# lightly-ai/lightly-train

Measured on NVIDIA B200. Metric: images/sec ViT-S/16 DINOv2 training step (2g+8l crops, bs64/GPU), higher is better.
Workload: dtype bf16

## Files before the change

lightly_train_b200/csrc/attention_tc.cu:

```cuda
#include <cuda.h>
#include "common.cuh"
#include "../../include/b200dino.h"

namespace b200 {
namespace attn_tc {

static constexpr int HD = 64;
static constexpr int BLOCK_Q = 128;
static constexpr int TILE_BYTES = BLOCK_Q * 128;
static constexpr float kLog2e = 1.4426950408889634f;

__device__ __forceinline__ uint64_t smem_desc(uint32_t smem_addr, uint32_t lbo_bytes, uint32_t sbo_bytes) {
  uint64_t d = 0;
  d |= (uint64_t)((smem_addr & 0x3FFFF) >> 4);
  d |= (uint64_t)((lbo_bytes >> 4) & 0x3FFF) << 16;
  d |= (uint64_t)((sbo_bytes >> 4) & 0x3FFF) << 32;
  d |= (uint64_t)1 << 46;
  d |= (uint64_t)2 << 61;
  return d;
}
__device__ __forceinline__ uint32_t instr_desc(int m, int n, int a_mn, int b_mn) {
  uint32_t d = 0;
  d |= 1u << 4;
  d |= 1u << 7;
// ... 791 lines not shown
    const uint32_t id_dq = instr_desc(BLOCK_Q, HD, 0, 1);
    for (int t = 0; t < n_tiles; ++t) {
      const uint32_t ph = t & 1;
      const uint64_t dQt_k = smem_desc(s0 + C::OFF_Q + t * TILE_BYTES, 16, 1024);
      const uint64_t dQt_mn = smem_desc(s0 + C::OFF_Q + t * TILE_BYTES, 64 * 128, 1024);
      const uint64_t dOt_k = smem_desc(s0 + C::OFF_DO + t * TILE_BYTES, 16, 1024);
      const uint64_t dOt_mn = smem_desc(s0 + C::OFF_DO + t * TILE_BYTES, 64 * 128, 1024);
      if (t > 0) {
        mbar_wait(bar_free, ph ^ 1);
        tc_fence_after();
      }
      if (elect_one_sync()) {
#pragma unroll
        for (int ks = 0; ks < 4; ++ks)
          umma_f16(tmem_base + C::TM_SDP, dQt_k + (uint64_t)(ks * 2), dK_kmaj + (uint64_t)(ks * 2), id_s, ks > 0 ? 1u : 0u);
        umma_commit(bar_s);
      }
      __syncwarp();
      mbar_wait(bar_p, ph);
      tc_fence_after();
      if (elect_one_sync()) {
#pragma unroll 1
        for (int mt = 0; mt < C::MT; ++mt)
#pragma unroll 1
          for (int ks = 0; ks < 8; ++ks)
            umma_f16(tmem_base + C::TM_DV + mt * 64, dP_mn + (uint64_t)((mt * 2 * TILE_BYTES + ks * 2048) >> 4),
                     dOt_mn + (uint64_t)((ks * 2048) >> 4), id_kv, (t > 0 || ks > 0) ? 1u : 0u);
#pragma unroll
        for (int ks = 0; ks < 4; ++ks)
          umma_f16(tmem_base + C::TM_SDP, dOt_k + (uint64_t)(ks * 2), dV_kmaj + (uint64_t)(ks * 2), id_s, ks > 0 ? 1u : 0u);
        umma_commit(bar_dp);
      }
      __syncwarp();
      mbar_wait(bar_ds, ph);
      tc_fence_after();
      if (elect_one_sync()) {
#pragma unroll 1
        for (int mt = 0; mt < C::MT; ++mt)
#pragma unroll 1
          for (int ks = 0; ks < 8; ++ks)
            umma_f16(tmem_base + C::TM_DK + mt * 64, dP_mn + (uint64_t)((mt * 2 * TILE_BYTES + ks * 2048) >> 4),
                     dQt_mn + (uint64_t)((ks * 2048) >> 4), id_kv, (t > 0 || ks > 0) ? 1u : 0u);
#pragma unroll 1
        for (int ks = 0; ks < NKV16; ++ks)
          umma_f16(tmem_base + C::TM_SDP, dP_kmaj + (uint64_t)(((ks >> 2) * TILE_BYTES + (ks & 3) * 32) >> 4),
                   dK_mn + (uint64_t)((ks * 2048) >> 4), id_dq, ks > 0 ? 1u : 0u);
        umma_commit(bar_dq);
      }
      __syncwarp();
    }
  } else {
    const int g = warp >> 2, q = warp & 3;
    const int r = q * 32 + lane;
    const uint32_t tL = tmem_base + ((uint32_t)(q * 32) << 16);
    const float sl2 = scale * kLog2e;
    uint8_t* sP = smem + C::OFF_P;
    if (g < C::QT) {
      const int m = g * BLOCK_Q + r;
      float L = 0.f, D = 0.f;
      if (m < rows_valid) {
        const int im = m / N;
        L = lse[((size_t)(b0 + im) * h + head) * N + (m - im * N)] * kLog2e;
        const uint4* po = reinterpret_cast<const uint4*>(outp + (row0 + m) * ld_out + head * HD);
        const uint4* pd = reinterpret_cast<const uint4*>(dout + (row0 + m) * ld_out + head * HD);
#pragma unroll
        for (int i = 0; i < 8; ++i) {
          const uint4 a = __ldg(po + i), c = __ldg(pd + i);
          const uint32_t aa[4] = {a.x, a.y, a.z, a.w}, cc[4] = {c.x, c.y, c.z, c.w};
#pragma unroll
          for (int j = 0; j < 4; ++j) {
            const float2 x = unpack_bf16x2(aa[j]), y = unpack_bf16x2(cc[j]);
            D = fmaf(x.x, y.x, D);
            D = fmaf(x.y, y.y, D);
          }
        }
      }
      sL[m] = L;
      sD[m] = D;
    }
    if (threadIdx.x < 192) sC[threadIdx.x] = 0.f;
    named_bar_sync(1, C::WORKERS * 32);
    for (int t = 0; t < n_tiles; ++t) {
      const uint32_t ph = t & 1;
      const int m = t * BLOCK_Q + r;
      const bool row_ok = m < rows_valid;
      const int klo = min(m / N, n_img - 1) * N, khi = klo + N;
      const float L = sL[m], D = sD[m];
      const int nfull = (G == 1) ? N / 16 : 0;
      mbar_wait(bar_s, ph);
      tc_fence_after();
      if (g == 0) bwd_p_pass<C::qb(0), C::qb(1)>(tL + C::TM_SDP, sP, r, row_ok, klo, khi, nfull, sl2, L);
      else if (g == 1) bwd_p_pass<C::qb(1), C::qb(2)>(tL + C::TM_SDP, sP, r, row_ok, klo, khi, nfull, sl2, L);
      else if (NG == 4 && g == 2) bwd_p_pass<C::qb(NG == 4 ? 2 : 0), C::qb(NG == 4 ? 3 : 1)>(tL + C::TM_SDP, sP, r, row_ok, klo, khi, nfull, sl2, L);
      else if (NG == 4) bwd_p_pass<C::qb(NG == 4 ? 3 : 0), C::qb(NG == 4 ? 4 : 1)>(tL + C::TM_SDP, sP, r, row_ok, klo, khi, nfull, sl2, L);
      fence_proxy_async();
      tc_fence_before();
      __syncwarp();
      if (lane == 0) mbar_arrive(bar_p);
      mbar_wait(bar_dp, ph);
      tc_fence_after();
      if (g == 0) bwd_ds_pass<C::qb(0), C::qb(1)>(tL + C::TM_SDP, sP, r, D);
      else if (g == 1) bwd_ds_pass<C::qb(1), C::qb(2)>(tL + C::TM_SDP, sP, r, D);
      else if (NG == 4 && g == 2) bwd_ds_pass<C::qb(NG == 4 ? 2 : 0), C::qb(NG == 4 ? 3 : 1)>(tL + C::TM_SDP, sP, r, D);
      else if (NG == 4) bwd_ds_pass<C::qb(NG == 4 ? 3 : 0), C::qb(NG == 4 ? 4 : 1)>(tL + C::TM_SDP, sP, r, D);
      fence_proxy_async();
      tc_fence_before();
      __syncwarp();
      if (lane == 0) mbar_arrive(bar_ds);
      if (g == 0 || (NG == 4 && g == 1)) {
        mbar_wait(bar_dq, ph);
        tc_fence_after();
        __nv_bfloat16* grow = dqkv + (row0 + m) * ld_dtok + head * HD;
        if (NG == 2) drain_tile(tL + C::TM_SDP, scale, row_ok, grow, colsum ? sC : nullptr, lane);
        else drain_cols32(tL + C::TM_SDP, g, scale, row_ok, grow, colsum ? sC : nullptr, lane);
        tc_fence_before();
        __syncwarp();
        if (lane == 0) mbar_arrive(bar_free);
      }
    }
    mbar_wait(bar_dq, (n_tiles - 1) & 1);
    tc_fence_after();
    if (NG == 2 && C::MT == 1) {
      const bool ok = r < rows_valid;
      __nv_bfloat16* base = dqkv + (row0 + r) * ld_dtok + head * HD + (size_t)(1 + g) * h * HD;
      drain_tile(tL + (g ? C::TM_DV : C::TM_DK), g ? 1.f : scale, ok, base, colsum ? sC + 64 + 64 * g : nullptr, lane);
    } else if (NG == 2) {
      const int key = g * BLOCK_Q + r;
      const bool ok = key < rows_valid;
      __nv_bfloat16* base = dqkv + (row0 + key) * ld_dtok + head * HD;
      drain_tile(tL + C::TM_DK + g * 64, scale, ok, base + (size_t)h * HD, colsum ? sC + 64 : nullptr, lane);
      drain_tile(tL + C::TM_DV + g * 64, 1.f, ok, base + (size_t)2 * h * HD, colsum ? sC + 128 : nullptr, lane);
    } else {
      const int mt = g & 1, is_v = g >> 1;
      const int key = mt * BLOCK_Q + r;
      const bool ok = key < rows_valid;
      __nv_bfloat16* base = dqkv + (row0 + key) * ld_dtok + head * HD + (size_t)(1 + is_v) * h * HD;
      drain_tile(tL + (is_v ? C::TM_DV : C::TM_DK) + mt * 64, is_v ? 1.f : scale, ok, base, colsum ? sC + 64 + 64 * is_v : nullptr, lane);
    }
    named_bar_sync(1, C::WORKERS * 32);
    if (colsum && threadIdx.x < 192) {
      const int part = threadIdx.x >> 6, d = threadIdx.x & 63;
      atomicAdd(colsum + (size_t)part * h * HD + head * HD + d, sC[threadIdx.x]);
    }
  }

  tc_fence_before();
  __syncthreads();
  if (warp == CTRL) {
    tc_fence_after();
    tmem_dealloc(tmem_base, C::TMEM_COLS);
  }
}

typedef CUresult (*PFN_encodeTiled)(CUtensorMap*, CUtensorMapDataType, cuuint32_t, void*, const cuuint64_t*, const cuuint64_t*,
                                    const cuuint32_t*, const cuuint32_t*, CUtensorMapInterleave, CUtensorMapSwizzle,
                                    CUtensorMapL2promotion, CUtensorMapFloatOOBfill);
static PFN_encodeTiled encode_fn() {
  static PFN_encodeTiled fn = nullptr;
  if (!fn) {
    void* p = nullptr;
    cudaDriverEntryPointQueryResult qres;
    if (cudaGetDriverEntryPoint("cuTensorMapEncodeTiled", &p, cudaEnableDefault, &qres) == cudaSuccess && p) fn = (PFN_encodeTiled)p;
  }
  return fn;
}
static int tmap_rows(CUtensorMap* tm, const void* base, long long rows, long long cols, long long ld, int box_rows) {
  PFN_encodeTiled enc = encode_fn();
  if (!enc) return B200_ERR_DRIVER;
  cuuint64_t dims[2] = {(cuuint64_t)cols, (cuuint64_t)rows};
  cuuint64_t strides[1] = {(cuuint64_t)ld * 2};
  cuuint32_t box[2] = {64u, (cuuint32_t)box_rows};
  cuuint32_t estr[2] = {1, 1};
  CUresult r = enc(tm, CU_TENSOR_MAP_DATA_TYPE_BFLOAT16, 2, const_cast<void*>(base), dims, strides, box, estr,
                   CU_TENSOR_MAP_INTERLEAVE_NONE, CU_TENSOR_MAP_SWIZZLE_128B, CU_TENSOR_MAP_L2_PROMOTION_L2_256B,
                   CU_TENSOR_MAP_FLOAT_OOB_FILL_NONE);
  return r == CUDA_SUCCESS ? B200_OK : B200_ERR_DRIVER;
}

template <int NKV16>
static int launch_fwd(const void* qkv, long long ld_tok, int B, int N, int G, int h, float scale, void* out, long long ld_out,
                      float* lse, cudaStream_t s) {
  using C = FwdCfg<NKV16>;
  CUtensorMap tmQ, tmKV;
  int rc = tmap_rows(&tmQ, qkv, (long long)B * N, 3LL * h * HD, ld_tok, BLOCK_Q);
  if (rc) return rc;
  rc = tmap_rows(&tmKV, qkv, (long long)B * N, 3LL * h * HD, ld_tok, C::NKV);
  if (rc) return rc;
  static bool attr = false;
  if (!attr) {
    if (cudaFuncSetAttribute(attn_fwd_tc_kernel<NKV16>, cudaFuncAttributeMaxDynamicSharedMemorySize, C::SMEM_BYTES) != cudaSuccess)
      return B200_ERR_CUDA;
    attr = true;
  }
  launch_kernel(attn_fwd_tc_kernel<NKV16>, ((B + G - 1) / G) * h, C::THREADS, C::SMEM_BYTES, s, tmQ, tmKV, B, N, G, h, scale, (__nv_bfloat16*)out,
                                                                                  ld_out, lse);
  B200_CHECK_LAUNCH();
  return B200_OK;
}

template <int NKV16>
static int launch_fwd7(const void* qkv, long long ld_tok, int B, int N, int G, int h, float scale, void* out, long long ld_out,
                       float* lse, cudaStream_t s) {
  using C = Fwd7Cfg<NKV16>;
  CUtensorMap tmQ, tmKV;
  int rc = tmap_rows(&tmQ, qkv, (long long)B * N, 3LL * h * HD, ld_tok, BLOCK_Q);
  if (rc) return rc;
  rc = tmap_rows(&tmKV, qkv, (long long)B * N, 3LL * h * HD, ld_tok, C::NKV);
  if (rc) return rc;
  static bool attr = false;
  if (!attr) {
    if (cudaFuncSetAttribute(attn_fwd_tc7_kernel<NKV16>, cudaFuncAttributeMaxDynamicSharedMemorySize, C::SMEM_BYTES) != cudaSuccess)
      return B200_ERR_CUDA;
    attr = true;
  }
  const int tiles = (G * N + BLOCK_Q - 1) / BLOCK_Q;
  launch_kernel(attn_fwd_tc7_kernel<NKV16>, ((B + G - 1) / G) * h * tiles, C::THREADS, C::SMEM_BYTES, s, tmQ, tmKV, B, N, G, h, tiles,
                scale, (__nv_bfloat16*)out, ld_out, lse);
  B200_CHECK_LAUNCH();
  return B200_OK;
}

template <int NKV16>
static int launch_fwd8(const void* qkv, long long ld_tok, int B, int N, int G, int h, float scale, void* out, long long ld_out,
                       float* lse, cudaStream_t s) {
  using C = Fwd7Cfg<NKV16>;
  CUtensorMap tmQ, tmKV;
  int rc = tmap_rows(&tmQ, qkv, (long long)B * N, 3LL * h * HD, ld_tok, BLOCK_Q);
  if (rc) return rc;
  rc = tmap_rows(&tmKV, qkv, (long long)B * N, 3LL * h * HD, ld_tok, C::NKV);
  if (rc) return rc;
  static bool attr = false;
  static int num_sms = 0;
  if (!attr) {
    if (cudaFuncSetAttribute(attn_fwd_tc8_kernel<NKV16>, cudaFuncAttributeMaxDynamicSharedMemorySize, C::SMEM_BYTES) != cudaSuccess)
      return B200_ERR_CUDA;
    int dev = 0;
    cudaGetDevice(&dev);
    cudaDeviceGetAttribute(&num_sms, cudaDevAttrMultiProcessorCount, dev);
    attr = true;
  }
  const int tiles = (G * N + BLOCK_Q - 1) / BLOCK_Q;
  const int total = ((B + G - 1) / G) * h * tiles;
  const int grid = total < 2 * num_sms ? total : 2 * num_sms;
  launch_kernel(attn_fwd_tc8_kernel<NKV16>, grid, C::THREADS, C::SMEM_BYTES, s, tmQ, tmKV, B, N, G, h, tiles, total, scale,
                (__nv_bfloat16*)out, ld_out, lse);
  B200_CHECK_LAUNCH();
  return B200_OK;
}

template <int NKV16, int NG>
static int launch_bwd(const void* qkv, long long ld_tok, const void* out, const void* dout, long long ld_out, const float* lse, int B,
                      int N, int G, int h, float scale, void* dqkv, long long ld_dtok, float* colsum, cudaStream_t s) {
  using C = BwdCfg<NKV16, NG>;
  CUtensorMap tmQ, tmKV, tmDO;
  int rc = tmap_rows(&tmQ, qkv, (long long)B * N, 3LL * h * HD, ld_tok, BLOCK_Q);
  if (rc) return rc;
  rc = tmap_rows(&tmKV, qkv, (long long)B * N, 3LL * h * HD, ld_tok, C::NKV);
  if (rc) return rc;
  rc = tmap_rows(&tmDO, dout, (long long)B * N, (long long)h * HD, ld_out, BLOCK_Q);
  if (rc) return rc;
  static bool attr = false;
  if (!attr) {
    if (cudaFuncSetAttribute(attn_bwd_tc_kernel<NKV16, NG>, cudaFuncAttributeMaxDynamicSharedMemorySize, C::SMEM_BYTES) != cudaSuccess)
      return B200_ERR_CUDA;
    attr = true;
  }
  launch_kernel(attn_bwd_tc_kernel<NKV16, NG>, ((B + G - 1) / G) * h, C::THREADS, C::SMEM_BYTES, s, tmQ, tmKV, tmDO, (const __nv_bfloat16*)out,
                                                                                  (const __nv_bfloat16*)dout, ld_out, lse, B, N, G, h,
                                                                                  scale, (__nv_bfloat16*)dqkv, ld_dtok, colsum);
  B200_CHECK_LAUNCH();
  return B200_OK;
}

}
}

extern "C" int b200_attention_fwd_tc(const void* qkv, long long ld_tok, int B, int N, int h, int head_dim, float scale, void* out,
                                     long long ld_out, float* lse, void* stream) {
  using namespace b200::attn_tc;
  if (!qkv || !out || B <= 0 || N <= 0 || h <= 0 || !(scale > 0.f)) return B200_ERR_INVALID_ARG;
  if (head_dim != HD || (ld_tok % 8) || (ld_out % 8) || ((uintptr_t)qkv & 15) || ((uintptr_t)out & 15)) return B200_ERR_UNSUPPORTED;
  if (N > 256) return B200_ERR_UNSUPPORTED;
  cudaStream_t s = (cudaStream_t)stream;
  static int sched = -1;
  if (sched < 0) {
    const char* e = std::getenv("B200_ATTN_FWD_SCHEDULE");
    sched = (e && (e[0] == '1' || e[0] == '7' || e[0] == '8')) ? e[0] - '0' : 8;
  }
  if (sched == 8) {
    if (N <= 128) return launch_fwd8<8>(qkv, ld_tok, B, N, 128 / N, h, scale, out, ld_out, lse, s);
    if (N <= 208) return launch_fwd8<13>(qkv, ld_tok, B, N, 1, h, scale, out, ld_out, lse, s);
    return launch_fwd8<16>(qkv, ld_tok, B, N, 1, h, scale, out, ld_out, lse, s);
  }
  if (sched == 7) {
    if (N <= 128) return launch_fwd7<8>(qkv, ld_tok, B, N, 128 / N, h, scale, out, ld_out, lse, s);
    if (N <= 208) return launch_fwd7<13>(qkv, ld_tok, B, N, 1, h, scale, out, ld_out, lse, s);
    return launch_fwd7<16>(qkv, ld_tok, B, N, 1, h, scale, out, ld_out, lse, s);
  }
  if (N <= 128) return launch_fwd<8>(qkv, ld_tok, B, N, 128 / N, h, scale, out, ld_out, lse, s);
  if (N <= 208) return launch_fwd<13>(qkv, ld_tok, B, N, 1, h, scale, out, ld_out, lse, s);
  return launch_fwd<16>(qkv, ld_tok, B, N, 1, h, scale, out, ld_out, lse, s);
}

extern "C" int b200_attention_bwd_tc(const void* qkv, long long ld_tok, const void* out, const void* dout, long long ld_out,
                                     const float* lse, int B, int N, int h, int head_dim, float scale, void* dqkv,
                                     long long ld_dtok, float* dqkv_colsum, void* stream) {
  using namespace b200::attn_tc;
  if (!qkv || !out || !dout || !lse || !dqkv || B <= 0 || N <= 0 || h <= 0 || !(scale > 0.f)) return B200_ERR_INVALID_ARG;
  if (head_dim != HD || (ld_tok % 8) || (ld_out % 8) || (ld_dtok % 8)) return B200_ERR_UNSUPPORTED;
  if (((uintptr_t)qkv & 15) || ((uintptr_t)out & 15) || ((uintptr_t)dout & 15) || ((uintptr_t)dqkv & 15)) return B200_ERR_UNSUPPORTED;
  if (N > 208) return B200_ERR_UNSUPPORTED;
  cudaStream_t s = (cudaStream_t)stream;
  static int groups = -1;
  if (groups < 0) {
    const char* e = std::getenv("B200_ATTN_BWD_GROUPS");
    groups = (e && e[0] == '2') ? 2 : 4;
  }
  if (N <= 128) return launch_bwd<8, 2>(qkv, ld_tok, out, dout, ld_out, lse, B, N, 128 / N, h, scale, dqkv, ld_dtok, dqkv_colsum, s);
  if (groups == 4) {
    return launch_bwd<13, 4>(qkv, ld_tok, out, dout, ld_out, lse, B, N, 1, h, scale, dqkv, ld_dtok, dqkv_colsum, s);
  }
  return launch_bwd<13, 2>(qkv, ld_tok, out, dout, ld_out, lse, B, N, 1, h, scale, dqkv, ld_dtok, dqkv_colsum, s);
}
```

lightly_train_b200/csrc/common.cuh:

```cuda
#pragma once
#include <cuda_runtime.h>
#include <cuda_bf16.h>
#include <stdint.h>

#define B200_OK 0
#define B200_ERR_INVALID_ARG (-1)
#define B200_ERR_UNSUPPORTED (-2)
#define B200_ERR_CUDA (-3)
#define B200_ERR_DRIVER (-4)

#define B200_CHECK_LAUNCH()                                     \
  do {                                                          \
    cudaError_t e__ = cudaGetLastError();                       \
    if (e__ != cudaSuccess) return B200_ERR_CUDA - (int)e__ * 16; \
  } while (0)

#include <cstdlib>
#include <utility>

namespace b200 {

__device__ __forceinline__ void pdl_launch_dependents() { asm volatile("griddepcontrol.launch_dependents;"); }
__device__ __forceinline__ void pdl_wait() { asm volatile("griddepcontrol.wait;" ::: "memory"); }
#define B200_PDL_SYNC()                \
  do {                                 \
    b200::pdl_launch_dependents();     \
    b200::pdl_wait();                  \
  } while (0)

inline bool pdl_enabled() {
  static int v = -1;
  if (v < 0) {
    const char* e = std::getenv("B200_PDL");
    v = (e && e[0] == '1') ? 1 : 0;
  }
  return v == 1;
}

template <typename... KArgs, typename... Args>
inline void launch_kernel(void (*kernel)(KArgs...), dim3 grid, dim3 block, size_t smem, cudaStream_t stream, Args&&... args) {
  cudaLaunchConfig_t cfg = {};
  cfg.gridDim = grid;
  cfg.blockDim = block;
  cfg.dynamicSmemBytes = smem;
  cfg.stream = stream;
  cudaLaunchAttribute attr[1];
  attr[0].id = cudaLaunchAttributeProgrammaticStreamSerialization;
  attr[0].val.programmaticStreamSerializationAllowed = 1;
  cfg.attrs = attr;
  cfg.numAttrs = pdl_enabled() ? 1 : 0;
  (void)cudaLaunchKernelEx(&cfg, kernel, static_cast<KArgs>(std::forward<Args>(args))...);
}

__device__ __forceinline__ uint32_t smem_u32(const void* p) {
  return (uint32_t)__cvta_generic_to_shared(p);
}

__device__ __forceinline__ void mbar_init(uint64_t* bar, uint32_t count) {
  asm volatile("mbarrier.init.shared::cta.b64 [%0], %1;" ::"r"(smem_u32(bar)), "r"(count));
}
__device__ __forceinline__ void mbar_expect_tx(uint64_t* bar, uint32_t bytes) {
  asm volatile("mbarrier.arrive.expect_tx.shared::cta.b64 _, [%0], %1;" ::"r"(smem_u32(bar)),
               "r"(bytes)
               : "memory");
}
__device__ __forceinline__ void mbar_arrive(uint64_t* bar) {
  asm volatile("mbarrier.arrive.shared::cta.b64 _, [%0];" ::"r"(smem_u32(bar)) : "memory");
}
__device__ __forceinline__ bool mbar_try_wait(uint64_t* bar, uint32_t parity) {
  uint32_t ok;
  asm volatile(
      "{\n"
      ".reg .pred p;\n"
      "mbarrier.try_wait.parity.shared::cta.b64 p, [%1], %2;\n"
      "selp.u32 %0, 1, 0, p;\n"
      "}\n"
      : "=r"(ok)
      : "r"(smem_u32(bar)), "r"(parity)
      : "memory");
  return ok != 0;
}
__device__ __forceinline__ void mbar_wait(uint64_t* bar, uint32_t parity) {
  uint32_t spins = 0;
  while (!mbar_try_wait(bar, parity)) {
    if (++spins > (1u << 26)) __trap();
  }
}
__device__ __forceinline__ void fence_barrier_init() {
  asm volatile("fence.mbarrier_init.release.cluster;" ::: "memory");
}
__device__ __forceinline__ void fence_proxy_async() {
  asm volatile("fence.proxy.async.shared::cta;" ::: "memory");
}

__device__ __forceinline__ void tma_prefetch_desc(const void* tm) {
  asm volatile("prefetch.tensormap [%0];" ::"l"(tm) : "memory");
}
__device__ __forceinline__ void tma_load_2d(void* smem_dst, const void* tm, uint64_t* bar, int c0,
                                            int c1) {
  asm volatile(
      "cp.async.bulk.tensor.2d.shared::cluster.global.tile.mbarrier::complete_tx::bytes "
      "[%0], [%1, {%3, %4}], [%2];" ::"r"(smem_u32(smem_dst)),
      "l"(tm), "r"(smem_u32(bar)), "r"(c0), "r"(c1)
      : "memory");
}

__device__ __forceinline__ bool elect_one_sync() {
  uint32_t pred;
  asm volatile(
      "{\n"
      ".reg .pred p;\n"
      "elect.sync _|p, 0xffffffff;\n"
      "selp.u32 %0, 1, 0, p;\n"
      "}\n"
      : "=r"(pred));
  return pred != 0;
}

__device__ __forceinline__ void prefetch_l2(const void* p) {
  asm volatile("prefetch.global.L2 [%0];" ::"l"(p));
}

__device__ __forceinline__ void tmem_alloc(uint32_t* smem_dst, uint32_t ncols) {
  asm volatile("tcgen05.alloc.cta_group::1.sync.aligned.shared::cta.b32 [%0], %1;" ::"r"(
                   smem_u32(smem_dst)),
               "r"(ncols));
}
__device__ __forceinline__ void tmem_relinquish() {
  asm volatile("tcgen05.relinquish_alloc_permit.cta_group::1.sync.aligned;" ::);
}
__device__ __forceinline__ void tmem_dealloc(uint32_t taddr, uint32_t ncols) {
  asm volatile("tcgen05.dealloc.cta_group::1.sync.aligned.b32 %0, %1;" ::"r"(taddr), "r"(ncols));
}
__device__ __forceinline__ void tc_fence_before() {
  asm volatile("tcgen05.fence::before_thread_sync;" ::: "memory");
}
__device__ __forceinline__ void tc_fence_after() {
  asm volatile("tcgen05.fence::after_thread_sync;" ::: "memory");
}
__device__ __forceinline__ void umma_f16(uint32_t tmem_d, uint64_t adesc, uint64_t bdesc,
                                         uint32_t idesc, uint32_t accumulate) {
  asm volatile(
      "{\n"
      ".reg .pred p;\n"
      "setp.ne.b32 p, %4, 0;\n"
      "tcgen05.mma.cta_group::1.kind::f16 [%0], %1, %2, %3, p;\n"
      "}\n" ::"r"(tmem_d),
      "l"(adesc), "l"(bdesc), "r"(idesc), "r"(accumulate)
      : "memory");
}
__device__ __forceinline__ void umma_f16_ts(uint32_t tmem_d, uint32_t tmem_a, uint64_t bdesc, uint32_t idesc, uint32_t accumulate) {
  asm volatile(
      "{\n"
      ".reg .pred p;\n"
      "setp.ne.b32 p, %4, 0;\n"
      "tcgen05.mma.cta_group::1.kind::f16 [%0], [%1], %2, %3, p;\n"
      "}\n" ::"r"(tmem_d),
      "r"(tmem_a), "l"(bdesc), "r"(idesc), "r"(accumulate)
      : "memory");
}
__device__ __forceinline__ void umma_commit(uint64_t* bar) {
  asm volatile("tcgen05.commit.cta_group::1.mbarrier::arrive::one.shared::cluster.b64 [%0];" ::"r"(
                   smem_u32(bar))
               : "memory");
}
__device__ __forceinline__ uint32_t cluster_ctarank() {
  uint32_t r;
  asm volatile("mov.u32 %0, %%cluster_ctarank;" : "=r"(r));
  return r;
}
__device__ __forceinline__ void cluster_sync_all() {
  asm volatile("barrier.cluster.arrive.release.aligned;\nbarrier.cluster.wait.acquire.aligned;" ::: "memory");
}
__device__ __forceinline__ uint32_t mapa_u32(uint32_t smem_addr, uint32_t rank) {
  uint32_t r;
  asm volatile("mapa.shared::cluster.u32 %0, %1, %2;" : "=r"(r) : "r"(smem_addr), "r"(rank));
  return r;
}
__device__ __forceinline__ void mbar_arrive_cluster(uint32_t cluster_addr) {
  asm volatile("mbarrier.arrive.shared::cluster.b64 _, [%0];" ::"r"(cluster_addr) : "memory");
}
__device__ __forceinline__ void tma_load_2d_2sm(void* smem_dst, const void* tm, uint32_t bar_cluster_addr, int c0, int c1) {
  asm volatile(
      "cp.async.bulk.tensor.2d.cta_group::2.shared::cluster.global.tile.mbarrier::complete_tx::bytes "
      "[%0], [%1, {%3, %4}], [%2];" ::"r"(smem_u32(smem_dst)),
      "l"(tm), "r"(bar_cluster_addr), "r"(c0), "r"(c1)
      : "memory");
}
__device__ __forceinline__ void tmem_alloc_2sm(uint32_t* smem_dst, uint32_t ncols) {
  asm volatile("tcgen05.alloc.cta_group::2.sync.aligned.shared::cta.b32 [%0], %1;" ::"r"(smem_u32(smem_dst)), "r"(ncols));
}
__device__ __forceinline__ void tmem_relinquish_2sm() {
  asm volatile("tcgen05.relinquish_alloc_permit.cta_group::2.sync.aligned;" ::);
}
__device__ __forceinline__ void tmem_dealloc_2sm(uint32_t taddr, uint32_t ncols) {
  asm volatile("tcgen05.dealloc.cta_group::2.sync.aligned.b32 %0, %1;" ::"r"(taddr), "r"(ncols));
}
__device__ __forceinline__ void umma_f16_2sm(uint32_t tmem_d, uint64_t adesc, uint64_t bdesc, uint32_t idesc,
                                             uint32_t accumulate) {
  asm volatile(
      "{\n"
      ".reg .pred p;\n"
      "setp.ne.b32 p, %4, 0;\n"
      "tcgen05.mma.cta_group::2.kind::f16 [%0], %1, %2, %3, p;\n"
      "}\n" ::"r"(tmem_d),
      "l"(adesc), "l"(bdesc), "r"(idesc), "r"(accumulate)
      : "memory");
}
__device__ __forceinline__ void umma_commit_2sm(uint64_t* bar, uint16_t cta_mask) {
  asm volatile("tcgen05.commit.cta_group::2.mbarrier::arrive::one.shared::cluster.multicast::cluster.b64 [%0], %1;" ::"r"(
                   smem_u32(bar)),
               "h"(cta_mask)
               : "memory");
}

__device__ __forceinline__ void tmem_ld_32x32(uint32_t taddr, uint32_t (&v)[32]) {
  asm volatile(
      "tcgen05.ld.sync.aligned.32x32b.x32.b32 "
      "{%0, %1, %2, %3, %4, %5, %6, %7, %8, %9, %10, %11, %12, %13, %14, %15, "
      "%16, %17, %18, %19, %20, %21, %22, %23, %24, %25, %26, %27, %28, %29, %30, %31}, [%32];"
      : "=r"(v[0]), "=r"(v[1]), "=r"(v[2]), "=r"(v[3]), "=r"(v[4]), "=r"(v[5]), "=r"(v[6]),
        "=r"(v[7]), "=r"(v[8]), "=r"(v[9]), "=r"(v[10]), "=r"(v[11]), "=r"(v[12]), "=r"(v[13]),
        "=r"(v[14]), "=r"(v[15]), "=r"(v[16]), "=r"(v[17]), "=r"(v[18]), "=r"(v[19]), "=r"(v[20]),
        "=r"(v[21]), "=r"(v[22]), "=r"(v[23]), "=r"(v[24]), "=r"(v[25]), "=r"(v[26]), "=r"(v[27]),
        "=r"(v[28]), "=r"(v[29]), "=r"(v[30]), "=r"(v[31])
      : "r"(taddr));
}
__device__ __forceinline__ void tmem_ld_32x16(uint32_t taddr, uint32_t (&v)[16]) {
  asm volatile(
      "tcgen05.ld.sync.aligned.32x32b.x16.b32 "
      "{%0, %1, %2, %3, %4, %5, %6, %7, %8, %9, %10, %11, %12, %13, %14, %15}, [%16];"
      : "=r"(v[0]), "=r"(v[1]), "=r"(v[2]), "=r"(v[3]), "=r"(v[4]), "=r"(v[5]), "=r"(v[6]), "=r"(v[7]), "=r"(v[8]),
        "=r"(v[9]), "=r"(v[10]), "=r"(v[11]), "=r"(v[12]), "=r"(v[13]), "=r"(v[14]), "=r"(v[15])
      : "r"(taddr));
}
__device__ __forceinline__ void tmem_ld_32x8(uint32_t taddr, uint32_t (&v)[8]) {
  asm volatile("tcgen05.ld.sync.aligned.32x32b.x8.b32 {%0, %1, %2, %3, %4, %5, %6, %7}, [%8];"
               : "=r"(v[0]), "=r"(v[1]), "=r"(v[2]), "=r"(v[3]), "=r"(v[4]), "=r"(v[5]), "=r"(v[6]), "=r"(v[7])
               : "r"(taddr));
}
__device__ __forceinline__ void tmem_ld_wait() {
  asm volatile("tcgen05.wait::ld.sync.aligned;" ::: "memory");
}
__device__ __forceinline__ void tmem_st_32x8(uint32_t taddr, const uint32_t (&v)[8]) {
  asm volatile("tcgen05.st.sync.aligned.32x32b.x8.b32 [%0], {%1, %2, %3, %4, %5, %6, %7, %8};" ::"r"(taddr), "r"(v[0]), "r"(v[1]),
               "r"(v[2]), "r"(v[3]), "r"(v[4]), "r"(v[5]), "r"(v[6]), "r"(v[7])
               : "memory");
}
__device__ __forceinline__ void tmem_st_wait() {
  asm volatile("tcgen05.wait::st.sync.aligned;" ::: "memory");
}

__device__ __forceinline__ float bf16_round(float x) {
  return __bfloat162float(__float2bfloat16_rn(x));
}
__device__ __forceinline__ uint32_t pack_bf16x2(float lo, float hi) {
  __nv_bfloat162 h = __floats2bfloat162_rn(lo, hi);
  return *reinterpret_cast<uint32_t*>(&h);
}
// ... 75 lines not shown
```

Before: 3437.

## Add persistent pipelined attention backward kernel with TMEM-resident P and dS

Adds a new persistent attention backward kernel, enabled by default, that loops over (image group, head) pairs with a grid capped at the SM count. It keeps P and dS in tensor memory for the TS-form MMAs, double-buffers LSE and D, prefetches the next pair's tiles to L2 with TMA, and uses separate drain warps to overlap the dK/dV/dQ writeback with the next tile's work. The aim is to cut launch and tail overhead and the serialization between softmax-gradient math and tensor-core work. The cost is a much more complex mbarrier protocol with more room for ordering bugs, and tighter TMEM and shared-memory budgets.

```diff
diff --git a/lightly_train_b200/csrc/attention_tc.cu b/lightly_train_b200/csrc/attention_tc.cu
--- a/lightly_train_b200/csrc/attention_tc.cu
+++ b/lightly_train_b200/csrc/attention_tc.cu
@@ -967,6 +967,426 @@
   }
 }
 
+template <int NKV16>
+struct Bwd2Cfg {
+  static constexpr int NKV = NKV16 * 16;
+  static constexpr bool SMALL = NKV <= 128;
+  static constexpr int MT = SMALL ? 1 : 2;
+  static constexpr int NG = SMALL ? 2 : 4;
+  static constexpr int Q_BYTES = NKV * 128;
+  static constexpr int OFF_Q = 0;
+  static constexpr int OFF_DO = Q_BYTES;
+  static constexpr int OFF_K = 2 * Q_BYTES;
+  static constexpr int OFF_V = OFF_K + MT * TILE_BYTES;
+  static constexpr int OFF_DS = OFF_V + MT * TILE_BYTES;
+  static constexpr int OFF_F = OFF_DS + 2 * MT * TILE_BYTES;
+  static constexpr int OFF_BAR = OFF_F + (4 * 256 + 192) * 4;
+  static constexpr int SMEM_BYTES = OFF_BAR + 128 + 1024;
+  static constexpr int WORKERS = 4 * NG;
+  static constexpr int DRAIN = WORKERS;
+  static constexpr int CTRL = WORKERS + 4;
+  static constexpr int THREADS = (WORKERS + 5) * 32;
+  static constexpr int CTAS_PER_SM = SMALL ? 2 : 1;
+  static constexpr int TP = 0;
+  static constexpr int TDP = (NKV / 2 + 15) / 16 * 16;
+  static constexpr int TDS = TDP;
+  static constexpr int TDK = (TDP + NKV / 2 + 31) / 32 * 32;
+  static constexpr int TDV = TDP + NKV;
+  static constexpr int TDQ = SMALL ? 0 : TDV + 64;
+  static constexpr int TMEM_COLS = SMALL ? 256 : 512;
+  __host__ __device__ static constexpr int qb(int g) { return (NKV16 * g + NG - 1) / NG; }
+  static_assert(TDK + 64 <= TDP + NKV && TDV + 64 <= TMEM_COLS && TDQ + 64 * MT <= TMEM_COLS, "TMEM column plan");
+  static_assert(SMALL ? TDQ + 64 <= TDP : TDQ >= TDV + 64, "dQ overlaps only P^T (packed) or nothing (global)");
+  static_assert(CTAS_PER_SM * SMEM_BYTES <= 232448, "shared memory");
+};
+
+template <int NT>
+__device__ __forceinline__ void quarter_bar_sync(int q) {
+  switch (q) {
+    case 0: asm volatile("bar.sync 1, %0;" ::"n"(NT) : "memory"); break;
+    case 1: asm volatile("bar.sync 2, %0;" ::"n"(NT) : "memory"); break;
+    case 2: asm volatile("bar.sync 3, %0;" ::"n"(NT) : "memory"); break;
+    default: asm volatile("bar.sync 4, %0;" ::"n"(NT) : "memory"); break;
+  }
+}
+
+template <int NKV16, int C0, int C1>
+__device__ __forceinline__ void bwd2_p_pass(uint32_t tL, int qq, const float* L, bool key_ok, int qlo, int qhi, int nfull, float sl2) {
+  using C = Bwd2Cfg<NKV16>;
+  constexpr int NC = C1 - C0;
+  uint32_t sv[NC * 8];
+  uint32_t buf[16];
+  tmem_ld_32x16(tL + C0 * 16, buf);
+#pragma unroll
+  for (int c = 0; c < NC; ++c) {
+    tmem_ld_wait();
+#pragma unroll
+    for (int i = 0; i < 8; ++i) sv[c * 8 + i] = pack_bf16x2(__uint_as_float(buf[2 * i]), __uint_as_float(buf[2 * i + 1]));
+    if (c + 1 < NC) tmem_ld_32x16(tL + (C0 + c + 1) * 16, buf);
+  }
+  tc_fence_before();
+  quarter_bar_sync<C::NG * 32>(qq);
+  tc_fence_after();
+  const float kb = key_ok ? 0.f : -INFINITY;
+#pragma unroll
+  for (int c = 0; c < NC; ++c) {
+    const int q0 = (C0 + c) * 16;
+    uint32_t pw[8];
+    if (C0 + c < nfull) {
+#pragma unroll
+      for (int i = 0; i < 8; ++i) {
+        const float2 ss = unpack_bf16x2(sv[c * 8 + i]);
+        const float2 ll = *reinterpret_cast<const float2*>(L + q0 + 2 * i);
+        pw[i] = pack_bf16x2(ex2_ftz(fmaf(ss.x, sl2, kb - ll.x)), ex2_ftz(fmaf(ss.y, sl2, kb - ll.y)));
+      }
+    } else {
+#pragma unroll
+      for (int i = 0; i < 8; ++i) {
+        const float2 ss = unpack_bf16x2(sv[c * 8 + i]);
+        const float2 ll = *reinterpret_cast<const float2*>(L + q0 + 2 * i);
+        const int q = q0 + 2 * i;
+        const float p0 = (key_ok && q >= qlo && q < qhi) ? ex2_ftz(fmaf(ss.x, sl2, -ll.x)) : 0.f;
+        const float p1 = (key_ok && q + 1 >= qlo && q + 1 < qhi) ? ex2_ftz(fmaf(ss.y, sl2, -ll.y)) : 0.f;
+        pw[i] = pack_bf16x2(p0, p1);
+      }
+    }
+    tmem_st_32x8(tL + C::TP + (C0 + c) * 8, pw);
+  }
+  tmem_st_wait();
+}
+
+template <int NKV16, int C0, int C1>
+__device__ __forceinline__ void bwd2_ds_pass(uint32_t tL, int qq, const float* Dq, uint8_t* sDS, int r) {
+  using C = Bwd2Cfg<NKV16>;
+  constexpr int NC = C1 - C0;
+  uint32_t dv[NC * 8];
+  uint32_t buf[16];
+  tmem_ld_32x16(tL + C::TDP + C0 * 16, buf);
+#pragma unroll
+  for (int c = 0; c < NC; ++c) {
+    tmem_ld_wait();
+#pragma unroll
+    for (int i = 0; i < 8; ++i) dv[c * 8 + i] = pack_bf16x2(__uint_as_float(buf[2 * i]), __uint_as_float(buf[2 * i + 1]));
+    if (c + 1 < NC) tmem_ld_32x16(tL + C::TDP + (C0 + c + 1) * 16, buf);
+  }
+  uint32_t pk[8];
+  tmem_ld_32x8(tL + C::TP + C0 * 8, pk);
+  tc_fence_before();
+  quarter_bar_sync<C::NG * 32>(qq);
+  tc_fence_after();
+#pragma unroll
+  for (int c = 0; c < NC; ++c) {
+    tmem_ld_wait();
+    uint32_t pc[8];
+#pragma unroll
+    for (int i = 0; i < 8; ++i) pc[i] = pk[i];
+    if (c + 1 < NC) tmem_ld_32x8(tL + C::TP + (C0 + c + 1) * 8, pk);
+    const int q0 = (C0 + c) * 16;
+    uint32_t dw[8];
+#pragma unroll
+    for (int i = 0; i < 8; ++i) {
+      const float2 dp = unpack_bf16x2(dv[c * 8 + i]);
+      const float2 pp = unpack_bf16x2(pc[i]);
+      const float2 dd = *reinterpret_cast<const float2*>(Dq + q0 + 2 * i);
+      dw[i] = pack_bf16x2(pp.x * (dp.x - dd.x), pp.y * (dp.y - dd.y));
+    }
+    tmem_st_32x8(tL + C::TDS + (C0 + c) * 8, dw);
+    uint8_t* slab = sDS + ((C0 + c) >> 2) * TILE_BYTES;
+    const int ch = ((C0 + c) & 3) * 2;
+    *reinterpret_cast<uint4*>(slab + swz(r, ch)) = make_uint4(dw[0], dw[1], dw[2], dw[3]);
+    *reinterpret_cast<uint4*>(slab + swz(r, ch + 1)) = make_uint4(dw[4], dw[5], dw[6], dw[7]);
+  }
+  tmem_st_wait();
+}
+
+template <int MT>
+__device__ __forceinline__ void bwd2_drain_dq(uint32_t tdq, int r, int rows_valid, float scale, __nv_bfloat16* dq_rows, long long ld_dtok,
+                                              float* cs, int lane, uint64_t* bar_dqfree) {
+#pragma unroll 1
+  for (int mq = 0; mq < MT; ++mq)
+    drain_tile(tdq + mq * 64, scale, mq * BLOCK_Q + r < rows_valid, dq_rows + (size_t)mq * BLOCK_Q * ld_dtok, cs, lane);
+  tc_fence_before();
+  __syncwarp();
+  if (lane == 0) mbar_arrive(bar_dqfree);
+}
+
+template <int NKV16>
+__global__ void __launch_bounds__(Bwd2Cfg<NKV16>::THREADS, Bwd2Cfg<NKV16>::CTAS_PER_SM)
+attn_bwd_tc2_kernel(const __grid_constant__ CUtensorMap tmQ, const __grid_constant__ CUtensorMap tmKV,
+                    const __grid_constant__ CUtensorMap tmDO, const __nv_bfloat16* __restrict__ outp,
+                    const __nv_bfloat16* __restrict__ dout, long long ld_out, const float* __restrict__ lse, int B, int N, int G,
+                    int h, int n_pairs, float scale, __nv_bfloat16* __restrict__ dqkv, long long ld_dtok, float* __restrict__ colsum) {
+  pdl_launch_dependents();
+  using C = Bwd2Cfg<NKV16>;
+  constexpr int MT = C::MT;
+  extern __shared__ uint8_t smem_raw[];
+  uint8_t* smem = reinterpret_cast<uint8_t*>((reinterpret_cast<uintptr_t>(smem_raw) + 1023) & ~(uintptr_t)1023);
+  float* sL = reinterpret_cast<float*>(smem + C::OFF_F);
+  float* sD = sL + 512;
+  float* sC = sD + 512;
+  uint64_t* bars = reinterpret_cast<uint64_t*>(smem + C::OFF_BAR);
+  uint64_t* bar_qd = bars + 0;
+  uint64_t* bar_kv = bars + 1;
+  uint64_t* bar_s = bars + 3;
+  uint64_t* bar_p = bars + 4;
+  uint64_t* bar_dp = bars + 5;
+  uint64_t* bar_ds = bars + 6;
+  uint64_t* bar_dk = bars + 7;
+  uint64_t* bar_kvfree = bars + 8;
+  uint64_t* bar_dqfree = bars + 9;
+  uint32_t* tmem_slot = reinterpret_cast<uint32_t*>(bars + 10);
+
+  const int warp = threadIdx.x >> 5, lane = threadIdx.x & 31;
+  if (threadIdx.x == 0) {
+    mbar_init(bar_qd, 1);
+    for (int kt = 0; kt < MT; ++kt) mbar_init(bar_kv + kt, 1);
+    mbar_init(bar_s, 1);
+    mbar_init(bar_p, C::WORKERS);
+    mbar_init(bar_dp, 1);
+    mbar_init(bar_ds, C::WORKERS);
+    mbar_init(bar_dk, 1);
+    mbar_init(bar_kvfree, 4);
+    mbar_init(bar_dqfree, 4);
+    fence_barrier_init();
+  }
+  if (threadIdx.x < 192) sC[threadIdx.x] = 0.f;
+  if (warp == C::CTRL) {
+    if (lane == 0) {
+      tma_prefetch_desc(&tmQ);
+      tma_prefetch_desc(&tmKV);
+      tma_prefetch_desc(&tmDO);
+    }
+    tmem_alloc(tmem_slot, C::TMEM_COLS);
+    tmem_relinquish();
+  }
+  tc_fence_before();
+  __syncthreads();
+  tc_fence_after();
+  pdl_wait();
+  const uint32_t tmem_base = *tmem_slot;
+  const int n_mine = (n_pairs - (int)blockIdx.x + (int)gridDim.x - 1) / (int)gridDim.x;
+  auto pair_coords = [h, G](int it, int& head, int& b0) {
+    const int w = blockIdx.x + it * gridDim.x;
+    head = w % h;
+    b0 = (w / h) * G;
+  };
+
+  if (warp == C::CTRL) {
+    const uint32_t s0 = smem_u32(smem);
+    const uint64_t dQ_k = smem_desc(s0 + C::OFF_Q, 16, 1024);
+    const uint64_t dO_k = smem_desc(s0 + C::OFF_DO, 16, 1024);
+    const uint64_t dQ_mn = smem_desc(s0 + C::OFF_Q, 64 * 128, 1024);
+    const uint64_t dO_mn = smem_desc(s0 + C::OFF_DO, 64 * 128, 1024);
+    const uint32_t id_s = instr_desc(BLOCK_Q, C::NKV, 0, 0);
+    const uint32_t id_ts = instr_desc(BLOCK_Q, HD, 0, 1);
+    const uint32_t id_dq = instr_desc(BLOCK_Q, HD, 1, 1);
+    auto load_qd = [&](int it) {
+      int head, b0;
+      pair_coords(it, head, b0);
+      mbar_expect_tx(bar_qd, 2 * C::Q_BYTES);
+      tma_load_2d(smem + C::OFF_Q, &tmQ, bar_qd, head * HD, b0 * N);
+      tma_load_2d(smem + C::OFF_DO, &tmDO, bar_qd, head * HD, b0 * N);
+    };
+    auto load_kv = [&](int it, int kt) {
+      int head, b0;
+      pair_coords(it, head, b0);
+      mbar_expect_tx(bar_kv + kt, 2 * TILE_BYTES);
+      tma_load_2d(smem + C::OFF_K + kt * TILE_BYTES, &tmKV, bar_kv + kt, (h + head) * HD, b0 * N + kt * BLOCK_Q);
+      tma_load_2d(smem + C::OFF_V + kt * TILE_BYTES, &tmKV, bar_kv + kt, (2 * h + head) * HD, b0 * N + kt * BLOCK_Q);
+    };
+    if (lane == 0 && n_mine > 0) {
+      load_qd(0);
+      for (int kt = 0; kt < MT; ++kt) load_kv(0, kt);
+    }
+    __syncwarp();
+    for (int it = 0; it < n_mine; ++it) {
+      for (int kt = 0; kt < MT; ++kt) {
+        const int j = it * MT + kt;
+        if (kt == 0) {
+          mbar_wait(bar_qd, it & 1);
+          if (lane == 0 && it + 1 < n_mine) {
+            int head, b0;
+            pair_coords(it + 1, head, b0);
+            tma_prefetch_2d(&tmQ, head * HD, b0 * N);
+            tma_prefetch_2d(&tmDO, head * HD, b0 * N);
+            for (int k2 = 0; k2 < MT; ++k2) {
+              tma_prefetch_2d(&tmKV, (h + head) * HD, b0 * N + k2 * BLOCK_Q);
+              tma_prefetch_2d(&tmKV, (2 * h + head) * HD, b0 * N + k2 * BLOCK_Q);
+            }
+          }
+          __syncwarp();
+        }
+        mbar_wait(bar_kv + kt, it & 1);
+        if (C::SMALL && it > 0) mbar_wait(bar_dqfree, (it - 1) & 1);
+        tc_fence_after();
+        if (elect_one_sync()) {
+          const uint64_t dK_k = smem_desc(s0 + C::OFF_K + kt * TILE_BYTES, 16, 1024);
+#pragma unroll
+          for (int ks = 0; ks < HD / 16; ++ks)
+            umma_f16(tmem_base, dK_k + (uint64_t)(ks * 2), dQ_k + (uint64_t)(ks * 2), id_s, ks > 0 ? 1u : 0u);
+          umma_commit(bar_s);
+        }
+        __syncwarp();
+        mbar_wait(bar_p, j & 1);
+        if (j > 0) mbar_wait(bar_kvfree, (j - 1) & 1);
+        tc_fence_after();
+        if (elect_one_sync()) {
+#pragma unroll 1
+          for (int ks = 0; ks < NKV16; ++ks)
+            umma_f16_ts(tmem_base + C::TDV, tmem_base + C::TP + ks * 8, dO_mn + (uint64_t)((ks * 2048) >> 4), id_ts, ks > 0 ? 1u : 0u);
+          const uint64_t dV_k = smem_desc(s0 + C::OFF_V + kt * TILE_BYTES, 16, 1024);
+#pragma unroll
+          for (int ks = 0; ks < HD / 16; ++ks)
+            umma_f16(tmem_base + C::TDP, dV_k + (uint64_t)(ks * 2), dO_k + (uint64_t)(ks * 2), id_s, ks > 0 ? 1u : 0u);
+          umma_commit(bar_dp);
+        }
+        __syncwarp();
+        mbar_wait(bar_ds, j & 1);
+        if (!C::SMALL && kt == 0 && it > 0) mbar_wait(bar_dqfree, (it - 1) & 1);
+        tc_fence_after();
+        if (elect_one_sync()) {
+#pragma unroll 1
+          for (int ks = 0; ks < NKV16; ++ks)
+            umma_f16_ts(tmem_base + C::TDK, tmem_base + C::TDS + ks * 8, dQ_mn + (uint64_t)((ks * 2048) >> 4), id_ts, ks > 0 ? 1u : 0u);
+          const uint64_t dK_mn = smem_desc(s0 + C::OFF_K + kt * TILE_BYTES, 64 * 128, 1024);
+#pragma unroll 1
+          for (int mq = 0; mq < MT; ++mq) {
+            const uint64_t dS_mn = smem_desc(s0 + C::OFF_DS + mq * 2 * TILE_BYTES, TILE_BYTES, 1024);
+#pragma unroll 1
+            for (int ks = 0; ks < 8; ++ks)
+              umma_f16(tmem_base + C::TDQ + mq * 64, dS_mn + (uint64_t)((ks * 2048) >> 4), dK_mn + (uint64_t)((ks * 2048) >> 4), id_dq,
+                       (kt > 0 || ks > 0) ? 1u : 0u);
+          }
+          umma_commit(bar_dk);
+        }
+        __syncwarp();
+        mbar_wait(bar_dk, j & 1);
+        if (lane == 0 && it + 1 < n_mine) {
+          load_kv(it + 1, kt);
+          if (kt == MT - 1) load_qd(it + 1);
+        }
+        __syncwarp();
+      }
+    }
+  } else if (warp < C::WORKERS) {
+    const int g = warp >> 2, qq = warp & 3;
+    const int r = qq * 32 + lane;
+    const uint32_t tL = tmem_base + ((uint32_t)(qq * 32) << 16);
+    const float sl2 = scale * kLog2e;
+    uint8_t* sDS = smem + C::OFF_DS;
+    for (int it = 0; it < n_mine; ++it) {
+      int head, b0;
+      pair_coords(it, head, b0);
+      const int n_img = min(G, B - b0);
+      const int rows_valid = n_img * N;
+      const size_t row0 = (size_t)b0 * N;
+      float* L = sL + (it & 1) * 256;
+      float* Dq = sD + (it & 1) * 256;
+      for (int m = threadIdx.x; m < C::NKV; m += C::WORKERS * 32) {
+        float l = 0.f, d = 0.f;
+        if (m < rows_valid) {
+          const int im = m / N;
+          l = lse[((size_t)(b0 + im) * h + head) * N + (m - im * N)] * kLog2e;
+          const uint4* po = reinterpret_cast<const uint4*>(outp + (row0 + m) * ld_out + head * HD);
+          const uint4* pd = reinterpret_cast<const uint4*>(dout + (row0 + m) * ld_out + head * HD);
+#pragma unroll
+          for (int i = 0; i < 8; ++i) {
+            const uint4 a = __ldg(po + i), c = __ldg(pd + i);
+            const uint32_t aa[4] = {a.x, a.y, a.z, a.w}, cc[4] = {c.x, c.y, c.z, c.w};
+#pragma unroll
+            for (int k = 0; k < 4; ++k) {
+              const float2 x = unpack_bf16x2(aa[k]), y = unpack_bf16x2(cc[k]);
+              d = fmaf(x.x, y.x, d);
+              d = fmaf(x.y, y.y, d);
+            }
+          }
+        }
+        L[m] = l;
+        Dq[m] = d;
+        if (it + 1 < n_mine) {
+          int head1, b1;
+          pair_coords(it + 1, head1, b1);
+          if (m < min(G, B - b1) * N) {
+            const int im = m / N;
+            prefetch_l2(lse + ((size_t)(b1 + im) * h + head1) * N + (m - im * N));
+            prefetch_l2(outp + ((size_t)b1 * N + m) * ld_out + head1 * HD);
+            prefetch_l2(dout + ((size_t)b1 * N + m) * ld_out + head1 * HD);
+          }
+        }
+      }
+      named_bar_sync(5, C::WORKERS * 32);
+      const int nfull = (G == 1) ? N / 16 : 0;
+      for (int kt = 0; kt < MT; ++kt) {
+        const int j = it * MT + kt;
+        const int key = kt * BLOCK_Q + r;
+        const bool key_ok = key < rows_valid;
+        const int qlo = min(key / N, n_img - 1) * N, qhi = qlo + N;
+        mbar_wait(bar_s, j & 1);
+        tc_fence_after();
+        if (g == 0) bwd2_p_pass<NKV16, C::qb(0), C::qb(1)>(tL, qq, L, key_ok, qlo, qhi, nfull, sl2);
+        else if (g == 1) bwd2_p_pass<NKV16, C::qb(1), C::qb(2)>(tL, qq, L, key_ok, qlo, qhi, nfull, sl2);
+        else if (C::NG == 4 && g == 2) bwd2_p_pass<NKV16, C::qb(C::NG == 4 ? 2 : 0), C::qb(C::NG == 4 ? 3 : 1)>(tL, qq, L, key_ok, qlo, qhi, nfull, sl2);
+        else if (C::NG == 4) bwd2_p_pass<NKV16, C::qb(C::NG == 4 ? 3 : 0), C::qb(C::NG == 4 ? 4 : 1)>(tL, qq, L, key_ok, qlo, qhi, nfull, sl2);
+        tc_fence_before();
+        __syncwarp();
+        if (lane == 0) mbar_arrive(bar_p);
+        mbar_wait(bar_dp, j & 1);
+        tc_fence_after();
+        if (g == 0) bwd2_ds_pass<NKV16, C::qb(0), C::qb(1)>(tL, qq, Dq, sDS, r);
+        else if (g == 1) bwd2_ds_pass<NKV16, C::qb(1), C::qb(2)>(tL, qq, Dq, sDS, r);
+        else if (C::NG == 4 && g == 2) bwd2_ds_pass<NKV16, C::qb(C::NG == 4 ? 2 : 0), C::qb(C::NG == 4 ? 3 : 1)>(tL, qq, Dq, sDS, r);
+        else if (C::NG == 4) bwd2_ds_pass<NKV16, C::qb(C::NG == 4 ? 3 : 0), C::qb(C::NG == 4 ? 4 : 1)>(tL, qq, Dq, sDS, r);
+        fence_proxy_async();
+        tc_fence_before();
+        __syncwarp();
+        if (lane == 0) mbar_arrive(bar_ds);
+      }
+    }
+  } else {
+    const int qq = warp & 3;
+    const int r = qq * 32 + lane;
+    const uint32_t tL = tmem_base + ((uint32_t)(qq * 32) << 16);
+    float* cs = colsum ? sC : nullptr;
+    for (int it = 0; it < n_mine; ++it) {
+      int head, b0;
+      pair_coords(it, head, b0);
+      const int rows_valid = min(G, B - b0) * N;
+      const size_t row0 = (size_t)b0 * N;
+      __nv_bfloat16* dq_rows = dqkv + (row0 + r) * ld_dtok + head * HD;
+      for (int kt = 0; kt < MT; ++kt) {
+        const int j = it * MT + kt;
+        mbar_wait(bar_dk, j & 1);
+        tc_fence_after();
+        if (C::SMALL) bwd2_drain_dq<MT>(tL + C::TDQ, r, rows_valid, scale, dq_rows, ld_dtok, cs, lane, bar_dqfree);
+        const int key = kt * BLOCK_Q + r;
+        __nv_bfloat16* base = dqkv + (row0 + key) * ld_dtok + head * HD;
+        drain_tile(tL + C::TDK, scale, key < rows_valid, base + (size_t)h * HD, cs ? cs + 64 : nullptr, lane);
+        drain_tile(tL + C::TDV, 1.f, key < rows_valid, base + (size_t)2 * h * HD, cs ? cs + 128 : nullptr, lane);
+        tc_fence_before();
+        __syncwarp();
+        if (lane == 0) mbar_arrive(bar_kvfree);
+      }
+      if (!C::SMALL) bwd2_drain_dq<MT>(tL + C::TDQ, r, rows_valid, scale, dq_rows, ld_dtok, cs, lane, bar_dqfree);
+      if (cs) {
+        named_bar_sync(6, 128);
+        const int t = threadIdx.x - C::DRAIN * 32;
+        for (int i = t; i < 192; i += 128) {
+          atomicAdd(colsum + (size_t)(i >> 6) * h * HD + head * HD + (i & 63), sC[i]);
+          sC[i] = 0.f;
+        }
+        named_bar_sync(6, 128);
+      }
+    }
+  }
+
+  tc_fence_before();
+  __syncthreads();
+  if (warp == C::CTRL) {
+    tc_fence_after();
+    tmem_dealloc(tmem_base, C::TMEM_COLS);
+  }
+}
+
 typedef CUresult (*PFN_encodeTiled)(CUtensorMap*, CUtensorMapDataType, cuuint32_t, void*, const cuuint64_t*, const cuuint64_t*,
                                     const cuuint32_t*, const cuuint32_t*, CUtensorMapInterleave, CUtensorMapSwizzle,
                                     CUtensorMapL2promotion, CUtensorMapFloatOOBfill);
@@ -1087,6 +1507,35 @@
   return B200_OK;
 }
 
+template <int NKV16>
+static int launch_bwd2(const void* qkv, long long ld_tok, const void* out, const void* dout, long long ld_out, const float* lse, int B,
+                       int N, int G, int h, float scale, void* dqkv, long long ld_dtok, float* colsum, cudaStream_t s) {
+  using C = Bwd2Cfg<NKV16>;
+  CUtensorMap tmQ, tmKV, tmDO;
+  int rc = tmap_rows(&tmQ, qkv, (long long)B * N, 3LL * h * HD, ld_tok, C::NKV);
+  if (rc) return rc;
+  rc = tmap_rows(&tmKV, qkv, (long long)B * N, 3LL * h * HD, ld_tok, BLOCK_Q);
+  if (rc) return rc;
+  rc = tmap_rows(&tmDO, dout, (long long)B * N, (long long)h * HD, ld_out, C::NKV);
+  if (rc) return rc;
+  static bool attr = false;
+  static int num_sms = 0;
+  if (!attr) {
+    if (cudaFuncSetAttribute(attn_bwd_tc2_kernel<NKV16>, cudaFuncAttributeMaxDynamicSharedMemorySize, C::SMEM_BYTES) != cudaSuccess)
+      return B200_ERR_CUDA;
+    int dev = 0;
+    cudaGetDevice(&dev);
+    cudaDeviceGetAttribute(&num_sms, cudaDevAttrMultiProcessorCount, dev);
+    attr = true;
+  }
+  const int pairs = ((B + G - 1) / G) * h;
+  const int grid = pairs < C::CTAS_PER_SM * num_sms ? pairs : C::CTAS_PER_SM * num_sms;
+  launch_kernel(attn_bwd_tc2_kernel<NKV16>, grid, C::THREADS, C::SMEM_BYTES, s, tmQ, tmKV, tmDO, (const __nv_bfloat16*)out,
+                (const __nv_bfloat16*)dout, ld_out, lse, B, N, G, h, pairs, scale, (__nv_bfloat16*)dqkv, ld_dtok, colsum);
+  B200_CHECK_LAUNCH();
+  return B200_OK;
+}
+
 }
 }
 
@@ -1131,6 +1580,15 @@
     const char* e = std::getenv("B200_ATTN_BWD_GROUPS");
     groups = (e && e[0] == '2') ? 2 : 4;
   }
+  static int sched = -1;
+  if (sched < 0) {
+    const char* e = std::getenv("B200_ATTN_BWD_SCHEDULE");
+    sched = (e && e[0] == '1') ? 1 : 3;
+  }
+  if (sched == 3) {
+    if (N <= 128) return launch_bwd2<8>(qkv, ld_tok, out, dout, ld_out, lse, B, N, 128 / N, h, scale, dqkv, ld_dtok, dqkv_colsum, s);
+    return launch_bwd2<13>(qkv, ld_tok, out, dout, ld_out, lse, B, N, 1, h, scale, dqkv, ld_dtok, dqkv_colsum, s);
+  }
   if (N <= 128) return launch_bwd<8, 2>(qkv, ld_tok, out, dout, ld_out, lse, B, N, 128 / N, h, scale, dqkv, ld_dtok, dqkv_colsum, s);
   if (groups == 4) {
     return launch_bwd<13, 4>(qkv, ld_tok, out, dout, ld_out, lse, B, N, 1, h, scale, dqkv, ld_dtok, dqkv_colsum, s);
diff --git a/lightly_train_b200/csrc/common.cuh b/lightly_train_b200/csrc/common.cuh
--- a/lightly_train_b200/csrc/common.cuh
+++ b/lightly_train_b200/csrc/common.cuh
@@ -105,6 +105,10 @@
       : "memory");
 }
 
+__device__ __forceinline__ void tma_prefetch_2d(const void* tm, int c0, int c1) {
+  asm volatile("cp.async.bulk.prefetch.tensor.2d.L2.global.tile [%0, {%1, %2}];" ::"l"(tm), "r"(c0), "r"(c1) : "memory");
+}
+
 __device__ __forceinline__ bool elect_one_sync() {
   uint32_t pred;
   asm volatile(
```

Result: no change. 3444 (median of 6 runs) (+0.2%).
